# danielmtzbarba/carlabev-env

Hardware: AMD Instinct MI355X
Metric: env-steps/sec (whole node) at N_envs x 128x128 semantic obs (higher is better)
Workload: dtype f64 state / u8 frames; 1 GPU; ego-only empty scene (rt_no_traffic_v1), 4096 envs/GPU, 128x128 semantic 6-class; config_id=2, envs_per_gpu=4096, global_envs=4096, obs_size=128, obs_mode=bev_semantic, parallelism=env-sharded x1

## Files before the change

carlabev_env_amd/_lib.py:

```python
from __future__ import annotations

import ctypes
import os

HERE = os.path.dirname(os.path.abspath(__file__))
LIB_PATH = os.environ.get("CBEV_LIB") or os.path.join(HERE, "libcbev.so")

_P = ctypes.c_void_p
_I = ctypes.c_int
_I64 = ctypes.c_int64

_lib = None


class CbevError(RuntimeError):
    pass


def lib():
    global _lib
    if _lib is not None:
        return _lib
    if not os.path.exists(LIB_PATH):
        raise CbevError(f"{LIB_PATH} not built; run `python -m carlabev_env_amd.build` (hipcc, gfx950)")
# ... 31 lines not shown
    L.cbev_reset_terminated.restype = _I
    L.cbev_final_frames.argtypes = [_P, _P, _I, _I, _I, _P, _P, _P, _P, _P, _P]
    L.cbev_final_frames.restype = _I
    L.cbev_bank_cursor.argtypes = [_P, _P]
    L.cbev_bank_cursor.restype = _I
    L.cbev_reset_counts.argtypes = [_P, _P, _I]
    L.cbev_reset_counts.restype = _I
    L.cbev_bank_stride.argtypes = [_I]
    L.cbev_bank_stride.restype = _I
    L.cbev_set_deferred_reset.argtypes = [_P, _I]
    L.cbev_set_deferred_reset.restype = _I
    L.cbev_reset_pending.argtypes = [_P]
    L.cbev_reset_pending.restype = _I
    L.cbev_set_split_step.argtypes = [_P, _I]
    L.cbev_set_split_step.restype = _I
    L.cbev_flush.argtypes = [_P]
    L.cbev_flush.restype = _I
    L.cbev_expand_obs.argtypes = [_P, _P, _I, _I, _I, _I, _I, _P, _P, _P]
    L.cbev_expand_obs.restype = _I
    L.cbev_expand_obs_typed.argtypes = [_P, _P, _I, _I, _I, _I, _I, _P, _I, _P, _P]
    L.cbev_expand_obs_typed.restype = _I
    L.cbev_expand_obs_heads.argtypes = [_P, _P, _I, _I, _P, _I, _I, _P, _I, _P, _P]
    L.cbev_expand_obs_heads.restype = _I
    L.cbev_unpack_obs.argtypes = [_P, _P, _I, _I, _I, _P, _P]
    L.cbev_unpack_obs.restype = _I
    L.cbev_pack_frames.argtypes = [_P, _P, _I, _P, _P]
    L.cbev_pack_frames.restype = _I
    L.cbev_unpack_frames.argtypes = [_P, _P, _I, _P, _P]
    L.cbev_unpack_frames.restype = _I
    L.cbev_vector_obs.argtypes = [_P, _P, _I, _P, _P]
# ... 27 lines not shown
def check(rc: int, what: str = "cbev call"):
    if rc != 0:
        msg = lib().cbev_last_error().decode("utf-8", "replace")
        raise CbevError(f"{what} failed ({rc}): {msg}")


EXPORTED_SYMBOLS = ("cbev_abi_version", "cbev_params_size", "cbev_layout_of", "cbev_field_names", "cbev_last_error",
                    "cbev_create", "cbev_destroy", "cbev_set_map", "cbev_step", "cbev_reset", "cbev_bank_frames",
                    "cbev_reset_frames", "cbev_reset_masked", "cbev_reset_terminated", "cbev_bank_cursor",
                    "cbev_reset_counts", "cbev_bank_stride",
                    "cbev_set_deferred_reset", "cbev_reset_pending", "cbev_flush",
                    "cbev_expand_obs", "cbev_vector_obs", "cbev_set_fov_mask", "cbev_set_obs_size", "cbev_resize_obs", "cbev_profile", "cbev_profile_read",
                    "cbev_profile_raster", "cbev_error_flags", "cbev_set_episode_stats", "cbev_episode_slot",
                    "cbev_wall_clock_hz", "cbev_termination_count", "cbev_pack_frames", "cbev_unpack_frames",
                    "cbev_expand_obs_typed", "cbev_unpack_obs", "cbev_set_split_step", "cbev_step_repeat",
                    "cbev_step_masked", "cbev_step_heads", "cbev_expand_obs_heads", "cbev_final_frames")

REPEAT_MAX = 64

OBS_F32, OBS_F16, OBS_U8, OBS_BITS = 0, 1, 2, 3

ERR_ACTION_INDEX = 1
ERR_RASTER_WINDOW = 2
ERR_RETREAT_ROUTE = 4
```

carlabev_env_amd/csrc/cbev.hip:

```cpp
#include <hip/hip_runtime.h>
#include <math.h>
#include <stdarg.h>
#include <stdio.h>
#include <stdlib.h>
#include <string.h>

#include <algorithm>
#include <string>
#include <type_traits>
#include <vector>

#include "../../include/cbev.h"
#include "cbev_device.h"

__constant__ SgTables c_sg;

__device__ __forceinline__ void d_set_target_speed_mps(DRec& r, int a, double s) {
  s = d_pymax(0.0, s);
  RAD(r, CBEV_AD_T_SPEED_MPS, a) = s;
  RAD(r, CBEV_AD_T_SPEED, a) = s / CB_MPP;
}

__device__ __forceinline__ void d_bset(DRec& r, int a, int st, double speed_mps) {
  RAI(r, CBEV_AI_BSTATE, a) = st;
// ... 2830 lines not shown
        for (int b = 0; b < 4; ++b)
          if ((tm >> b) & 1u) *(uint32_t*)(g + o + 4 * b) = *(const uint32_t*)(l + o + 4 * b);
      }
    } else {
      const int w = j - nhd - nhi;
      *(uint32_t*)(g + K.L.vis + 4 * w) = *(const uint32_t*)(l + 16 * p.n0 + (K.L.vis - K.L.raw_x) + 4 * w);
    }
  }
}

template <bool WHOLE, EgoGate GATE = EgoGate::None, bool FIRST = false>
__device__ __forceinline__ void ego_tail(uint8_t* lds, uint8_t* __restrict__ recs, int n, int ne, int st_rb,
                                         int st_n0, int st_n, int st_raw_x, const KArgs& K,
                                         double* __restrict__ reward_out, uint8_t* __restrict__ term_out,
                                         uint8_t* __restrict__ trunc_out, int32_t* __restrict__ cause_out,
                                         float* __restrict__ info_out, EgoCarry& C, uint64_t frozen_in = 0ull) {
  constexpr bool GATED = GATE != EgoGate::None;
  constexpr bool ACCUM = GATE == EgoGate::Term || (GATE == EgoGate::Mask && !FIRST);
  const int e0 = staged_env0(blockIdx.x, ne, n);
  const int ne_eff = min(ne, n - e0);
  if (ne_eff <= 0) return;
  const EgoPack pk = ego_pack(K.L);
  const int nslot = WHOLE && K.C.actor_cap == 0 ? 2 : 1;
  const CollScratchLayout SL = coll_scratch_layout(K.C, K.L.vis_words);
  const EgoLds M = ego_lds(lds, nslot, ne, pk, SL);
  uint8_t* const scr = M.scr;
  HeroPre* const pre = M.pre;
  const int* const rrow = M.rrow;
  const int tid = threadIdx.x;
  const int lane = tid & 63, wave = __builtin_amdgcn_readfirstlane(tid >> 6);
  const cbev_params& P = K.P;
// ... 172 lines not shown
        }
        {
          double rx_ = ax - x, ry_ = ay - y;
          double rvx = avx - hvx, rvy = avy - hvy;
          double nrm = sqrt(rx_ * rx_ + ry_ * ry_);
          double rel = (rvx * rx_ + rvy * ry_) / (nrm + 1e-6);
          if (!(rel >= 0)) ts = fabs(nrm / rel);
        }
      }
      ((double*)(scr + k * SL.bytes + SL.ttcc))[a] = tc;
      ((double*)(scr + k * SL.bytes + SL.ttcs))[a] = ts;
    }
  }
  __syncthreads();
  CBEV_STAMP(1, 1);
  if (tid < ne_eff && !(GATED && ((frozen >> tid) & 1ull))) {
    const DRec r = rec(tid);
    CollPre cp = coll_reduce_serial(scr + tid * SL.bytes, SL, r.hi[CBEV_HI_NACT], r.hi[CBEV_HI_NRAW]);
    cp.spx = C.spx;
    cp.spy = C.spy;
    double rsum = 0.0;
    if (ACCUM) rsum = reward_out[e0 + tid];
    collide_env(K, r, e0 + tid, cp, reward_out, term_out, trunc_out, cause_out, info_out);
    if (ACCUM) reward_out[e0 + tid] = rsum + r.hd[CBEV_HD_REWARD];
    if (r.hi[CBEV_HI_TERM]) K.tcount[e0 + tid] = tc0 + 1u;
  } else if (GATE == EgoGate::Mask && FIRST && tid < ne_eff) {
    reward_out[e0 + tid] = 0.0;
  }
  __syncthreads();
  CBEV_STAMP(1, 2);
  if (!WHOLE) {
    ego_tail_out(lds, recs, e0, ne_eff, K, pk);
    CBEV_STAMP(1, 3);
    return;
  }
  if (GATED) {
    ego_stage_out_live(lds, recs, e0, ne_eff, K, pk, frozen);
    return;
  }
  ego_stage_out(slot, recs, e0, ne_eff, K, pk);
  if (C.rest_k >= 0) *(uint4*)(recs + (int64_t)(e0 + C.rest_k) * rb + C.rest_o) = C.rest_v;
  const int rsA = (int)((K.L.vis - K.L.cx) / 16), rsB0 = (int)(K.L.vis / 16) + pk.nvis;
  const int rpp = rsA + (int)(rb / 16) - rsB0, nres = __popcll(rbits);
  for (int q = threadIdx.x + 256; q < nres * rpp; q += 256) {
    const int k = nth_set_bit(rbits, q / rpp), c = q % rpp;
    const int o = c < rsA ? (int)K.L.cx + 16 * c : 16 * (rsB0 + c - rsA);
    *(uint4*)(recs + (int64_t)(e0 + k) * rb + o) = *(const uint4*)(src(k) + o);
// ... 69 lines not shown
  extern __shared__ __align__(16) uint8_t lds[];
  ego_mask_body<FIRST, false>(lds, recs, n, ne, st_rb, st_n0, st_n, st_raw_x, K, actions, active, reward_out, term_out,
                              trunc_out, cause_out, info_out, nullptr, 0);
}
__global__ __launch_bounds__(256) void k_ego_heads(uint8_t* __restrict__ recs, int n, int ne, int st_rb, int st_n0,
                                                   int st_n, int st_raw_x, KArgs K, const void* __restrict__ actions,
                                                   const uint8_t* __restrict__ active, double* __restrict__ reward_out,
                                                   uint8_t* __restrict__ term_out, uint8_t* __restrict__ trunc_out,
                                                   int32_t* __restrict__ cause_out, float* __restrict__ info_out,
                                                   uint8_t* __restrict__ heads, int n_frames) {
  extern __shared__ __align__(16) uint8_t lds[];
  ego_mask_body<true, true>(lds, recs, n, ne, st_rb, st_n0, st_n, st_raw_x, K, actions, active, reward_out, term_out,
                            trunc_out, cause_out, info_out, heads, n_frames);
}

__global__ __launch_bounds__(256) void k_ego_head(uint8_t* __restrict__ recs, int n, int ne, int st_rb, KArgs K,
                                                  const void* __restrict__ actions) {
  __shared__ double sh_pre[2][3][64];
  __shared__ float sh_act[3][64];
  CBEV_STAMP(0, 0);
  const int e0 = staged_env0(blockIdx.x, ne, n);
  const int ne_eff = min(ne, n - e0);
  if (ne_eff <= 0) return;
  const int tid = threadIdx.x;
  const int lane = tid & 63, wave = __builtin_amdgcn_readfirstlane(tid >> 6);
  const bool on = lane < ne_eff;
  const int e = e0 + (on ? lane : 0);
  const int vw = K.L.vis_words;
  const bool fold = K.rmask != nullptr;
  const uint8_t* const mp = fold ? K.rmask + e : recs;
  uint32_t mb = 0u, tc = 0u;
  double hd[CBEV_HD_COUNT] = {};
  int32_t hi[CBEV_HI_COUNT] = {};
  DRec r{};
  r.hd = hd;
  r.hi = hi;
  constexpr int NIN = 7;
  auto load_in = [&](const uint8_t* src, double* in) {
    const double* g = (const double*)(src + K.L.hd);
#pragma unroll
    for (int k = 0; k < 4; ++k) in[k] = g[CBEV_HD_X + k];
    in[4] = g[CBEV_HD_ACC];
    in[5] = g[CBEV_HD_TSPEED];
    in[6] = g[CBEV_HD_T];
  };
  auto chain = [&](int pass, const double* in) {
// ... 2 lines not shown
    hd[CBEV_HD_ACC] = in[4];
    hd[CBEV_HD_TSPEED] = in[5];
    hd[CBEV_HD_T] = in[6];
    HeroPre hp;
    hp.cyaw = sh_pre[pass][0][lane];
    hp.syaw = sh_pre[pass][1][lane];
    hp.tdelta = sh_pre[pass][2][lane];
    const float act3[3] = {sh_act[0][lane], sh_act[1][lane], sh_act[2][lane]};
    hero_env_phys(K, r, e, actions, hp, act3);
    hero_env_render_setup(K, r);
  };
  double in0[NIN] = {}, in1[NIN] = {}, v0 = 0.0, v1 = 0.0;
  float sa = 0.0f;
  const uint8_t* const own = recs + (int64_t)e * st_rb;
  if (wave == 0) {
    if (on) {
      load_in(own, in0);
      mb = *mp;
      tc = K.tcount[e];
      d_sincos(in0[2], &sh_pre[0][1][lane], &sh_pre[0][0][lane]);
    }
  } else if (wave == 1) {
    if (on) {
      v0 = ((const double*)(own + K.L.hd))[CBEV_HD_V];
      mb = *mp;
      tc = K.tcount[e];
      float g, b;
      d_decode_action(K, actions, e, &g, &sa, &b);
      sh_act[0][lane] = g;
      sh_act[1][lane] = sa;
      sh_act[2][lane] = b;
      sh_pre[0][2][lane] = hero_tan_delta(v0, sa);
    }
  } else {
    mb = *mp;
    tc = K.tcount[e];
    for (int q = tid - 128; q < ne_eff * vw; q += 128) {
      const int k = q / vw, w = q - k * vw;
      uint8_t* g = recs + (int64_t)(e0 + k) * st_rb + K.L.vis;
      const uint32_t v = ((const uint32_t*)g)[w];
      if (!(fold && K.rmask[e0 + k] != 0)) ((uint32_t*)g)[vw + w] = v;
    }
  }
  __syncthreads();
  CBEV_STAMP(0, 1);
  const bool reset = fold && on && mb != 0u;
  const uint64_t rbits = __ballot(reset);
  const int row = reset ? bank_row_of(e, tc, K.rstride, K.rn_bank) : 0;
  const uint8_t* const bank = K.rbank + (int64_t)row * st_rb;
  if (wave == 0 && reset) load_in(bank, in1);
  if (wave == 1 && reset) v1 = ((const double*)(bank + K.L.hd))[CBEV_HD_V];
  if (wave == 0 && on && !reset) chain(0, in0);
  if (rbits != 0ull) {
    if (wave == 0) {
      if (reset) {
#pragma unroll
        for (int k = 0; k < NIN; ++k) asm volatile("" : "+v"(in1[k]));
        d_sincos(in1[2], &sh_pre[1][1][lane], &sh_pre[1][0][lane]);
      }
    } else if (wave == 1) {
      if (reset) sh_pre[1][2][lane] = hero_tan_delta(v1, sa);
    } else {
      const int np = st_rb / 16, total = __popcll(rbits) * np;
      const int d0 = (int)K.L.vis + 4 * vw, d1 = d0 + 4 * vw;
      auto piece = [&](int q, const uint8_t** b, uint8_t** g, int* o) {
        const int j = q < total ? q / np : 0, k = nth_set_bit(rbits, j);
        *o = 16 * (q - j * np);
        *b = K.rbank + (int64_t)__shfl(row, k) * st_rb + *o;
        *g = recs + (int64_t)(e0 + k) * st_rb + *o;
      };
      auto by_word = [&](const uint8_t* b, uint8_t* g, int o) {
        for (int w = 0; w < 16; w += 4)
          *(uint32_t*)(g + w) = *(const uint32_t*)(b + w - (o + w >= d0 && o + w < d1 ? 4 * vw : 0));
      };
      for (int base = tid - 128; base - (tid - 128) < total; base += 256) {
        const uint8_t *b0, *b1;
        uint8_t *g0, *g1;
        int o0, o1;
        piece(base, &b0, &g0, &o0);
        piece(base + 128, &b1, &g1, &o1);
        const bool a0 = base < total, a1 = base + 128 < total;
        const bool w0 = o0 + 16 <= d0 || o0 >= d1, w1 = o1 + 16 <= d0 || o1 >= d1;
        uint4 x0 = make_uint4(0, 0, 0, 0), x1 = x0;
        if (a0 && w0) x0 = *(const uint4*)b0;
        if (a1 && w1) x1 = *(const uint4*)b1;
        if (a0 && w0) *(uint4*)g0 = x0;
        if (a1 && w1) *(uint4*)g1 = x1;
        if (a0 && !w0) by_word(b0, g0, o0);
        if (a1 && !w1) by_word(b1, g1, o1);
      }
    }
    __syncthreads();
    if (wave == 0 && reset) chain(1, in1);
  }
  CBEV_STAMP(0, 2);
  if (wave == 0 && on) {
    if (reset) {
      hi[CBEV_HI_RS_FAST] |= (row + 1) << 1;
      if (K.stats != nullptr) K.stats[e].t0 = (double)wall_clock64();
    }
    uint8_t* g = recs + (int64_t)e * st_rb;
    double* ohd = (double*)(g + K.L.hd);
    int32_t* ohi = (int32_t*)(g + K.L.hi);
#pragma unroll
    for (int k = 0; k < 8; k += 2) *(double2*)(ohd + CBEV_HD_X + k) = make_double2(hd[CBEV_HD_X + k], hd[CBEV_HD_X + k + 1]);
    ohd[CBEV_HD_ACC] = hd[CBEV_HD_ACC];
    *(double2*)(ohd + CBEV_HD_U_GAS) = make_double2(hd[CBEV_HD_U_GAS], hd[CBEV_HD_U_STEER]);
    *(double2*)(ohd + CBEV_HD_U_BRAKE) = make_double2(hd[CBEV_HD_U_BRAKE], hd[CBEV_HD_U_DELTA]);
    ohd[CBEV_HD_T] = hd[CBEV_HD_T];
#pragma unroll
    for (int k = CBEV_HI_RS_XMIN; k <= CBEV_HI_RS_FAST; ++k) ohi[k] = hi[k];
  }
  CBEV_STAMP(0, 3);
}
constexpr int HEAD_NE_DEFAULT = 16;
static_assert(CBEV_HD_X % 2 == 0 && CBEV_HD_U_GAS % 2 == 0 && CBEV_HD_U_BRAKE == CBEV_HD_U_GAS + 2 &&
                  CBEV_HD_U_DELTA == CBEV_HD_U_GAS + 3,
              "k_ego_head stores X .. V1 and U_* as 16-byte pieces");

struct TailArgs {
  int ntail;
  int ne, rb, n0, np, raw_x;
  double* reward;
  uint8_t* term;
  uint8_t* trunc;
  int32_t* cause;
  float* info;
};

struct RasterArgs {
  KArgs K;
  uint8_t* recs;
  int n;
  uint8_t* frames;
  TailArgs T;
};
template <int G>
__global__ __launch_bounds__(kRasterNT)
__attribute__((amdgpu_waves_per_eu(Tiles<G>::wgs_per_cu * kRasterNT / 256 > 8 ? 8 : Tiles<G>::wgs_per_cu * kRasterNT / 256)))
void k_raster(RasterArgs A) {
  extern __shared__ __align__(16) uint8_t lds[];
  if constexpr (G > 1) {
    if ((int)blockIdx.x < A.T.ntail) {
      const RasterArgs M = *(const RasterArgs*)__builtin_amdgcn_kernarg_segment_ptr();
      const TailArgs& T = M.T;
      EgoCarry C;
      ego_tail<false>(lds, M.recs, M.n, T.ne, T.rb, T.n0, T.np, T.raw_x, M.K, T.reward, T.term, T.trunc, T.cause,
                      T.info, C);
      return;
    }
  }
  const KArgs& K = A.K;
  uint8_t* __restrict__ const recs = A.recs;
  uint8_t* __restrict__ const frames = A.frames;
  const int n = A.n;
  const TailArgs& T = A.T;
  CBEV_STAMP(2, 0);
  int e, t;
  xcd_tile_of_wg((int)blockIdx.x - T.ntail, n, Tiles<G>::T, &e, &t);
  if (e >= n) return;
  const int64_t SS = (int64_t)K.P.size * K.P.size;
  const DRec r = bind_rec(recs + (int64_t)e * K.L.record_bytes, K.L, K.C);
  const RasterJob J = raster_job<false, G>(K, r);
// ... 416 lines not shown
  int defer_reset;
  struct {
    int on;
    void* records;
    int n;
    const uint8_t* mask;
    const void* bank;
    int n_bank;
    const uint8_t* bank_frames;
    uint8_t* frames;
    int n_frames;
    void* stream;
  } pend;
  const uint8_t* last_term;
  int last_n;
};

static int ego_ne_for(int per_env, int actor_cap) {
  const int budget = 128 * 1024;
  const char* v = getenv("CBEV_EGO_NE");
  int ne = v ? atoi(v) : (actor_cap <= 16 ? 16 : actor_cap <= 32 ? 8 : 4);
  ne = ne >= 64 ? 64 : ne >= 32 ? 32 : ne >= 16 ? 16 : ne >= 8 ? 8 : 4;
  while (ne > 4 && ne * per_env > budget) ne >>= 1;
  return ne * per_env > budget ? 0 : ne;
}

static int head_ne_for() {
  const char* v = getenv("CBEV_HEAD_NE");
  const int ne = v ? atoi(v) : HEAD_NE_DEFAULT;
  return ne >= 64 ? 64 : ne >= 32 ? 32 : ne >= 16 ? 16 : ne >= 8 ? 8 : 4;
// ... 174 lines not shown
  do {                                                                                                \
    if (!(c)->map_dev) return set_err(CBEV_ESTATE, "cbev_set_map not called");                        \
    if ((n) <= 0) return CBEV_OK;                                                                     \
    if ((c)->stats && (n) > (c)->ep_n)                                                                \
      return set_err(CBEV_EINVAL, "n %d exceeds the %d envs of the episode stats", (n), (c)->ep_n); \
  } while (0)

struct StepRun {
  KArgs K;
  hipStream_t s;
  hipEvent_t* ev;
};
static int step_begin(cbev_ctx* c, int n, uint8_t* term, void* stream, StepRun* R) {
  R->s = (hipStream_t)stream;
  R->K = kargs(c);
  c->last_term = term;
  c->last_n = n;
  if (n > c->seq_n) c->seq_n = n;
  if (c->stats) {
    const int slot = (int)(c->step_count % c->ep_ring), next = (slot + 1) % c->ep_ring;
    R->K.ep_rows = c->ep_rows + (int64_t)slot * c->ep_n * CBEV_EP_COUNT;
    R->K.ep_count = c->ep_counts + slot;
    R->K.ep_count_next = c->ep_counts + next;
    R->K.ep_cap = c->ep_n;
    c->step_count += 1;
  }
  R->ev = c->prof_on && c->prof_n < CBEV_PROF_MAX ? c->prof_ev + 4 * c->prof_n++ : nullptr;
  if (R->ev) HIP_TRY(hipEventRecord(R->ev[0], R->s));
  return CBEV_OK;
}
// ... 69 lines not shown
    return set_err(CBEV_EINVAL, "record layout: the k_ego staging ranges are not contiguous");
  if (ego_ne == 0)
    return set_err(CBEV_EINVAL, "k_ego stages 4 records per workgroup: %d bytes each do not fit its LDS budget",
                   per_env);
  HIP_TRY(hipSetDevice(device));
  cbev_ctx* c = (cbev_ctx*)calloc(1, sizeof(cbev_ctx));
  c->P = P;
  c->C = *caps;
  c->L = lay;
  c->device = device;
  c->ego_ne = ego_ne;
  c->ego_lb = ego_ne * per_env;
  c->tail_ne = tail_ne_for(P, *caps, lay, ego_ne);
  c->split = c->tail_ne > 0;
  c->head_ne = head_ne_for();
  SgTables T;
  build_sg_tables(&T);
  hipError_t e = hipMemcpyToSymbol(HIP_SYMBOL(c_sg), &T, sizeof T);
  if (e == hipSuccess) e = hipMalloc(&c->lut_dev, 64 * sizeof(uint32_t));
  if (e == hipSuccess) e = hipMalloc(&c->err_dev, sizeof(int32_t));
  if (e == hipSuccess) e = hipMemset(c->err_dev, 0, sizeof(int32_t));
  if (e == hipSuccess) e = hipMalloc(&c->nterm_dev, sizeof(unsigned long long));
  if (e == hipSuccess) e = hipMemset(c->nterm_dev, 0, sizeof(unsigned long long));
  const size_t seq_bytes = (size_t)CBEV_RESET_MASK_MAX_N * sizeof(uint32_t);
  if (e == hipSuccess) e = hipMalloc(&c->seq_dev, seq_bytes);
  if (e == hipSuccess) e = hipMemset(c->seq_dev, 0, seq_bytes);
  if (e == hipSuccess) {
    int khz = 0;
    e = hipDeviceGetAttribute(&khz, hipDeviceAttributeWallClockRate, device);
    c->tick_s = khz > 0 ? 1.0 / (1000.0 * khz) : 0.0;
  }
  if (e == hipSuccess) {
    const uint32_t pal[16] = CBEV_PALETTE_RGB;
    e = hipMemcpyToSymbol(HIP_SYMBOL(c_palette_rgb), pal, sizeof pal);
  }
  c->obs_h = c->obs_w = P.size;
  if (e == hipSuccess)
    e = hipFuncSetAttribute((const void*)k_ego, hipFuncAttributeMaxDynamicSharedMemorySize, c->ego_lb);
  if (e == hipSuccess)
    e = hipFuncSetAttribute((const void*)k_ego_rep, hipFuncAttributeMaxDynamicSharedMemorySize, c->ego_lb);
  if (e == hipSuccess)
// ... 135 lines not shown
void cbev_destroy(cbev_ctx* c) {
  if (!c) return;
  c->pend.on = 0;
  (void)hipSetDevice(c->device);
  if (c->prof_ev) {
    for (int i = 0; i < 4 * CBEV_PROF_MAX; ++i) (void)hipEventDestroy(c->prof_ev[i]);
    free(c->prof_ev);
  }
  if (c->map_dev) (void)hipFree(c->map_dev);
  if (c->map8_dev) (void)hipFree(c->map8_dev);
  if (c->map8T_dev) (void)hipFree(c->map8T_dev);
  if (c->lut_dev) (void)hipFree(c->lut_dev);
  if (c->err_dev) (void)hipFree(c->err_dev);
  if (c->nterm_dev) (void)hipFree(c->nterm_dev);
  if (c->seq_dev) (void)hipFree(c->seq_dev);
  if (c->area_dev) (void)hipFree(c->area_dev);
  if (c->fov_dev) (void)hipFree(c->fov_dev);
  free(c);
}

int cbev_set_map(cbev_ctx* c, const uint8_t* map_host, int64_t bytes) {
  if (!c || !map_host) return set_err(CBEV_EINVAL, "null argument");
  CBEV_FLUSH(c);
  const int64_t need = (int64_t)c->P.map_pitch * c->P.render_h;
  if (bytes != need) return set_err(CBEV_EINVAL, "map bytes %lld != pitch*render_h %lld", (long long)bytes, (long long)need);
  const int W = c->P.render_w, H = c->P.render_h, pitch = c->P.map_pitch;
  for (int64_t i = 0; i < need; ++i)
    if (map_host[i] > 15) return set_err(CBEV_EINVAL, "class id %d > 15 at byte %lld", map_host[i], (long long)i);
  const int np = ((W + 1) / 2 + 63) & ~63;
  std::vector<uint8_t> packed((size_t)np * H, 0);
// ... 28 lines not shown
  HIP_TRY(hipMemcpy(c->map8T_dev, map8T.data(), (size_t)p8T * W, hipMemcpyHostToDevice));
  c->p8T = p8T;
  return CBEV_OK;
}

int cbev_step(cbev_ctx* c, void* records, int n, const void* actions, uint8_t* frames, double* reward, uint8_t* term,
              uint8_t* trunc, int32_t* cause, float* info, void* stream) {
  if (!c || !records || !actions || !frames || !reward || !term || !trunc || !cause)
    return set_err(CBEV_EINVAL, "null argument");
  CBEV_STEP_CHECKS(c, n);
  const int64_t stride = (int64_t)n * c->P.size * c->P.size;
  const int64_t off = c->pend.on ? frames - c->pend.frames : 0;
  const bool fold = c->pend.on && records == c->pend.records && n == c->pend.n && off >= 0 && off % stride == 0 &&
                    off / stride < c->pend.n_frames && fold_ok(c, n);
  if (!fold) CBEV_FLUSH(c);
  StepRun R;
  const int rc = step_begin(c, n, term, stream, &R);
  if (rc != CBEV_OK) return rc;
  if (fold) {
    R.K.rmask = c->pend.mask;
    R.K.rbank = (const uint8_t*)c->pend.bank;
    R.K.rbank_frames = c->pend.bank_frames;
    R.K.rring = c->pend.frames;
    R.K.rring_stride = stride;
    R.K.rn_bank = c->pend.n_bank;
    R.K.rn_frames = c->pend.n_frames;
    R.K.rslot = (int)(off / stride);
    R.K.rstride = bank_stride(c->pend.n_bank);
    c->pend.on = 0;
  }
  launch_actors(c, actors_kernel(c->C), R, records, n);
  if (R.ev) HIP_TRY(hipEventRecord(R.ev[1], R.s));
  TailArgs T{};
  if (c->split) {
    hipLaunchKernelGGL(k_ego_head, dim3((n + c->head_ne - 1) / c->head_ne), dim3(256), 0, R.s, (uint8_t*)records, n,
                       c->head_ne, (int)c->L.record_bytes, R.K, actions);
    const EgoPack pk = ego_pack(c->L);
    T = TailArgs{((n + c->tail_ne - 1) / c->tail_ne + 7) & ~7, c->tail_ne, (int)c->L.record_bytes, pk.n0, pk.n,
                 (int)c->L.raw_x, reward, term, trunc, cause, info};
  } else {
    launch_ego(c, k_ego, R, records, n, actions, reward, term, trunc, cause, info);
  }
  if (R.ev) HIP_TRY(hipEventRecord(R.ev[2], R.s));
  launch_raster(c, CBEV_BY_SIZE(k_raster, c->P.size), n, T.ntail, R.s,
                RasterArgs{R.K, (uint8_t*)records, n, frames, T});
  return step_end(R);
}

enum StepKind { STEP_REPEAT, STEP_MASKED, STEP_HEADS };
struct StepChain {
  StepKind kind;
  const uint8_t *active, *prev_frames;
  uint8_t* heads;
  int n_frames;
// ... 99 lines not shown
  if (n <= 0) return CBEV_OK;
  KArgs K = kargs(c);
  const size_t lb = raster_lds_bytes(c->P);
  hipStream_t s = (hipStream_t)stream;
  const int grid = n < RESET_WGS ? n : RESET_WGS;
  hipLaunchKernelGGL(CBEV_BY_SIZE(k_reset, c->P.size), dim3(grid), dim3(256), lb, s, K, (uint8_t*)records, n,
                     (const uint8_t*)bank, n_bank, mask, bank_idx, bank_offset, frames, n_frames);
  HIP_TRY(hipGetLastError());
  return CBEV_OK;
}

int cbev_bank_frames(cbev_ctx* c, const void* bank, int n_bank, uint8_t* frames, void* stream) {
  if (!c || !bank || !frames) return set_err(CBEV_EINVAL, "null argument");
  CBEV_FLUSH(c);
  if (!c->map_dev) return set_err(CBEV_ESTATE, "cbev_set_map not called");
  if (n_bank <= 0) return CBEV_OK;
  KArgs K = kargs(c);
  const size_t lb = raster_lds_bytes(c->P);
  hipStream_t s = (hipStream_t)stream;
  const int grid = n_bank < RESET_WGS ? n_bank : RESET_WGS;
  hipLaunchKernelGGL(CBEV_BY_SIZE(k_bank_frames, c->P.size), dim3(grid), dim3(256), lb, s, K, (const uint8_t*)bank,
                     n_bank, frames);
  HIP_TRY(hipGetLastError());
  return CBEV_OK;
}

int cbev_reset_frames(cbev_ctx* c, void* records, int n, const void* bank, int n_bank, const uint8_t* mask,
                      const int32_t* bank_idx, int bank_offset, const uint8_t* bank_frames, uint8_t* frames,
                      int n_frames, void* stream) {
  if (!c || !records || !bank || !bank_frames || !frames) return set_err(CBEV_EINVAL, "null argument");
// ... 18 lines not shown
  if (n > CBEV_RESET_MASK_MAX_N) return set_err(CBEV_EINVAL, "n %d exceeds %d", n, CBEV_RESET_MASK_MAX_N);
  if (n <= 0) return CBEV_OK;
  CBEV_FLUSH(c);
  return launch_reset_mask(c, records, n, mask, bank, n_bank, bank_frames, frames, n_frames, stream);
}

static int launch_reset_mask(cbev_ctx* c, void* records, int n, const uint8_t* mask, const void* bank, int n_bank,
                             const uint8_t* bank_frames, uint8_t* frames, int n_frames, void* stream) {
  KArgs K = kargs(c);
  const int SS = c->P.size * c->P.size;
  const int64_t ppe = reset_pieces((int64_t)SS) + reset_pieces(c->L.record_bytes);
  const int64_t pieces = (int64_t)n * ppe;
  const int grid = pieces >= RESET_MASK_WGS ? RESET_MASK_WGS : (int)pieces;
  const int upt = reset_mask_upt(n);
  if (n > c->seq_n) c->seq_n = n;
  hipLaunchKernelGGL(k_reset_mask, dim3(grid), dim3(256), reset_mask_lds(n), (hipStream_t)stream, n, n_bank,
                     bank_stride(n_bank), (int)c->L.record_bytes, SS, n_frames, upt, mask, c->seq_dev,
                     (uint8_t*)records, (const uint8_t*)bank, bank_frames, frames, K);
  HIP_TRY(hipGetLastError());
  return CBEV_OK;
}

int cbev_reset_terminated(cbev_ctx* c, void* records, int n, const void* bank, int n_bank, const uint8_t* bank_frames,
                          uint8_t* frames, int n_frames, void* stream) {
  if (!c) return set_err(CBEV_EINVAL, "null argument");
  if (c->last_n == 0) return set_err(CBEV_ESTATE, "cbev_reset_terminated before any cbev_step");
  if (n != c->last_n) return set_err(CBEV_EINVAL, "n %d != the %d envs of the last cbev_step", n, c->last_n);
  if (c->defer_reset && fold_ok(c, n)) {
    if (!records || !bank || !bank_frames || !frames) return set_err(CBEV_EINVAL, "null argument");
    if (n_bank <= 0) return set_err(CBEV_EINVAL, "empty bank");
// ... 18 lines not shown
  if (!c) return set_err(CBEV_EINVAL, "null argument");
  if (!on) CBEV_FLUSH(c);
  c->defer_reset = on != 0;
  return CBEV_OK;
}

int cbev_reset_pending(const cbev_ctx* c) { return c && c->pend.on ? 1 : 0; }

int cbev_set_split_step(cbev_ctx* c, int on) {
  if (!c) return set_err(CBEV_EINVAL, "null argument");
  if (on && c->tail_ne == 0)
    return set_err(CBEV_EINVAL, "the split step is not supported at size %d with these capacities: k_ego's tail "
                                "does not fit k_raster's registers or its %zu bytes of LDS",
                   c->P.size, raster_lds_bytes(c->P));
  c->split = on != 0;
  return CBEV_OK;
}

int cbev_flush(cbev_ctx* c) {
  if (!c) return set_err(CBEV_EINVAL, "null argument");
  return flush_pending(c);
}

int cbev_bank_cursor(cbev_ctx* c, int64_t* cursor) {
  if (!c || !cursor) return set_err(CBEV_EINVAL, "null argument");
  CBEV_FLUSH(c);
  HIP_TRY(hipSetDevice(c->device));
  HIP_TRY(hipDeviceSynchronize());
  std::vector<uint32_t> v((size_t)c->seq_n);
  if (c->seq_n > 0) HIP_TRY(hipMemcpy(v.data(), c->seq_dev, v.size() * sizeof(uint32_t), hipMemcpyDeviceToHost));
// ... 382 lines not shown
```

carlabev_env_amd/csrc/cbev_device.h:

```cpp
#pragma once

#include <hip/hip_runtime.h>
#include <stdint.h>

#include "../../include/cbev_layout.h"

#define CB_DT 0.1
#define CB_WHEELBASE 2.9
#define CB_MPP 0.3125
#define CB_PI 3.141592653589793

struct KArgs {
  cbev_params P;
  cbev_caps C;
  cbev_layout L;
  const uint8_t* map;
  int npitch;
  const uint8_t* map8;
  int p8;
  const uint8_t* map8T;
  int p8T;
  const uint32_t* fov;
  int32_t* err;
  unsigned long long* nterm;
  cbev_episode_stats* stats;
  double* ep_rows;
  int32_t* ep_count;
  int32_t* ep_count_next;
  int ep_cap;
  double tick_s;
  uint32_t* tcount;
  const uint8_t* rmask;
  const uint8_t* rbank;
  const uint8_t* rbank_frames;
  uint8_t* rring;
  int64_t rring_stride;
  int rn_bank, rn_frames, rslot;
  uint32_t rstride;
};

__device__ __forceinline__ int d_map_texel(const KArgs& K, int x, int y) {
  return (K.map[(int64_t)y * K.npitch + (x >> 1)] >> ((x & 1) << 2)) & 15;
}

struct SgTables {
  double conv[6][11];
  double left[6][5][11];
  double right[6][5][11];
};
extern __constant__ SgTables c_sg;

struct DRec {
  double* hd;
// ... 225 lines not shown
```

include/cbev.h:

```cpp
#ifndef CBEV_H
#define CBEV_H

#include <stdint.h>

#include "cbev_layout.h"

#ifdef __cplusplus
extern "C" {
#endif

#define CBEV_ABI_VERSION 7

typedef struct cbev_ctx cbev_ctx;

enum { CBEV_OK = 0, CBEV_EINVAL = -1, CBEV_EHIP = -2, CBEV_ESTATE = -3 };

int cbev_abi_version(void);
int cbev_params_size(void);
int cbev_layout_of(const cbev_caps* caps, cbev_layout* out);
const char* cbev_field_names(int group);
const char* cbev_last_error(void);

int cbev_create(const cbev_params* params, const cbev_caps* caps, int device, cbev_ctx** out);
void cbev_destroy(cbev_ctx* ctx);
// ... 40 lines not shown
                      const uint8_t* bank_frames, uint8_t* frames, int n_frames, void* stream);
int cbev_reset_terminated(cbev_ctx* ctx, void* records, int n, const void* bank, int n_bank,
                          const uint8_t* bank_frames, uint8_t* frames, int n_frames, void* stream);
int cbev_final_frames(cbev_ctx* ctx, const uint8_t* ring, int n, int n_frames, int head, const uint8_t* heads,
                      const uint8_t* mask, uint8_t* out, int32_t* out_env, int32_t* out_count, void* stream);

int cbev_bank_cursor(cbev_ctx* ctx, int64_t* cursor);
int cbev_reset_counts(cbev_ctx* ctx, uint32_t* counts_host, int n);
int cbev_bank_stride(int n_bank);
int cbev_set_deferred_reset(cbev_ctx* ctx, int on);
int cbev_reset_pending(const cbev_ctx* ctx);
int cbev_flush(cbev_ctx* ctx);

int cbev_set_split_step(cbev_ctx* ctx, int on);

int cbev_expand_obs(cbev_ctx* ctx, const uint8_t* ring, int n, int n_frames, int head, int kind, int n_channels,
                    const uint32_t* channel_lut_host, void* out, void* stream);

#define CBEV_OBS_F32 0
#define CBEV_OBS_F16 1
#define CBEV_OBS_U8 2
#define CBEV_OBS_BITS 3
int cbev_expand_obs_typed(cbev_ctx* ctx, const uint8_t* ring, int n, int n_frames, int head, int kind, int n_channels,
                          const uint32_t* channel_lut_host, int out_dtype, void* out, void* stream);
int cbev_expand_obs_heads(cbev_ctx* ctx, const uint8_t* ring, int n, int n_frames, const uint8_t* heads, int kind,
                          int n_channels, const uint32_t* channel_lut_host, int out_dtype, void* out, void* stream);
int cbev_unpack_obs(cbev_ctx* ctx, const uint8_t* packed, int rows, int pixels, int out_dtype, void* out, void* stream);

int cbev_vector_obs(cbev_ctx* ctx, const void* records, int n, float* out, void* stream);

// ... 21 lines not shown
```

Baseline: 119.9 million env-steps/s.

## Preview reset-bank ego state in the tail so the next head skips reload

When an env terminates in the split-step tail, the tail now writes the bank row's ego head state (x, y, yaw, v, acc, target speed, t) into a 64-byte per-env preview slot tagged with the step serial, and a wave touches the bank row to warm the cache. On the next folded reset, k_ego_head<true> checks the tag and row, runs the kinematic chain directly from the previewed inputs, and skips the bank load and second sync for those envs. Head-state words are left out of the bank copy for all resets. This adds a preview buffer, atomic counters, template dispatch and tag bookkeeping, and depends on the preview staying consistent with the pending bank.

```diff
diff --git a/carlabev_env_amd/_lib.py b/carlabev_env_amd/_lib.py
--- a/carlabev_env_amd/_lib.py
+++ b/carlabev_env_amd/_lib.py
@@ -69,6 +69,10 @@
     L.cbev_reset_pending.restype = _I
     L.cbev_set_split_step.argtypes = [_P, _I]
     L.cbev_set_split_step.restype = _I
+    L.cbev_set_reset_preview.argtypes = [_P, _I]
+    L.cbev_set_reset_preview.restype = _I
+    L.cbev_reset_preview_counts.argtypes = [_P, _P]
+    L.cbev_reset_preview_counts.restype = _I
     L.cbev_flush.argtypes = [_P]
     L.cbev_flush.restype = _I
     L.cbev_expand_obs.argtypes = [_P, _P, _I, _I, _I, _I, _I, _P, _P, _P]
@@ -126,7 +130,8 @@
                     "cbev_profile_raster", "cbev_error_flags", "cbev_set_episode_stats", "cbev_episode_slot",
                     "cbev_wall_clock_hz", "cbev_termination_count", "cbev_pack_frames", "cbev_unpack_frames",
                     "cbev_expand_obs_typed", "cbev_unpack_obs", "cbev_set_split_step", "cbev_step_repeat",
-                    "cbev_step_masked", "cbev_step_heads", "cbev_expand_obs_heads", "cbev_final_frames")
+                    "cbev_step_masked", "cbev_step_heads", "cbev_expand_obs_heads", "cbev_final_frames",
+                    "cbev_set_reset_preview", "cbev_reset_preview_counts")
 
 REPEAT_MAX = 64
 
diff --git a/carlabev_env_amd/csrc/cbev.hip b/carlabev_env_amd/csrc/cbev.hip
--- a/carlabev_env_amd/csrc/cbev.hip
+++ b/carlabev_env_amd/csrc/cbev.hip
@@ -2868,7 +2868,8 @@
                                          int st_n0, int st_n, int st_raw_x, const KArgs& K,
                                          double* __restrict__ reward_out, uint8_t* __restrict__ term_out,
                                          uint8_t* __restrict__ trunc_out, int32_t* __restrict__ cause_out,
-                                         float* __restrict__ info_out, EgoCarry& C, uint64_t frozen_in = 0ull) {
+                                         float* __restrict__ info_out, EgoCarry& C, uint64_t frozen_in = 0ull,
+                                         const PvArgs* pvw = nullptr) {
   constexpr bool GATED = GATE != EgoGate::None;
   constexpr bool ACCUM = GATE == EgoGate::Term || (GATE == EgoGate::Mask && !FIRST);
   const int e0 = staged_env0(blockIdx.x, ne, n);
@@ -3071,6 +3072,8 @@
   }
   __syncthreads();
   CBEV_STAMP(1, 1);
+  int trow1 = 0;
+  uint32_t touched = 0u;
   if (tid < ne_eff && !(GATED && ((frozen >> tid) & 1ull))) {
     const DRec r = rec(tid);
     CollPre cp = coll_reduce_serial(scr + tid * SL.bytes, SL, r.hi[CBEV_HI_NACT], r.hi[CBEV_HI_NRAW]);
@@ -3080,14 +3083,47 @@
     if (ACCUM) rsum = reward_out[e0 + tid];
     collide_env(K, r, e0 + tid, cp, reward_out, term_out, trunc_out, cause_out, info_out);
     if (ACCUM) reward_out[e0 + tid] = rsum + r.hd[CBEV_HD_REWARD];
-    if (r.hi[CBEV_HI_TERM]) K.tcount[e0 + tid] = tc0 + 1u;
+    if (r.hi[CBEV_HI_TERM]) {
+      K.tcount[e0 + tid] = tc0 + 1u;
+      if (GATE == EgoGate::None && pvw != nullptr && K.rbank != nullptr && pvw->tag != 0u) {
+        const int row = bank_row_of(e0 + tid, tc0 + 1u, K.rstride, K.rn_bank);
+        const double* g = (const double*)(K.rbank + (int64_t)row * st_rb + K.L.hd);
+        RPreview* const pv = pvw->pv + (e0 + tid);
+        const double x = g[CBEV_HD_X], y = g[CBEV_HD_Y], yaw = g[CBEV_HD_YAW], v = g[CBEV_HD_V];
+        const double acc = g[CBEV_HD_ACC], ts = g[CBEV_HD_TSPEED], t = g[CBEV_HD_T];
+        double2* const o = (double2*)pv;
+        o[0] = make_double2(x, y);
+        o[1] = make_double2(yaw, v);
+        o[2] = make_double2(acc, ts);
+        union {
+          uint32_t u[2];
+          double d;
+        } w;
+        w.u[0] = (uint32_t)row + 1u;
+        w.u[1] = pvw->tag;
+        o[3] = make_double2(t, w.d);
+        trow1 = row + 1;
+      }
+    }
   } else if (GATE == EgoGate::Mask && FIRST && tid < ne_eff) {
     reward_out[e0 + tid] = 0.0;
+  }
+  if (!WHOLE && GATE == EgoGate::None && wave == 0 && pvw != nullptr && K.rbank != nullptr && pvw->tag != 0u) {
+    uint32_t t0 = 0u, t1 = 0u;
+    for (uint64_t tb = __ballot(trow1 != 0); tb != 0ull; tb &= tb - 1ull) {
+      const int row = __shfl(trow1, __builtin_ctzll(tb)) - 1;
+      const uint8_t* const b = K.rbank + (int64_t)row * st_rb;
+      t0 |= *(const uint32_t*)(b + min(128 * lane, st_rb - 4));
+      t1 |= *(const uint32_t*)(b + st_rb - 4);
+      for (int o = 128 * (64 + lane); o < st_rb; o += 128 * 64) t1 |= *(const uint32_t*)(b + o);
+    }
+    touched = t0 | t1;
   }
   __syncthreads();
   CBEV_STAMP(1, 2);
   if (!WHOLE) {
     ego_tail_out(lds, recs, e0, ne_eff, K, pk);
+    asm volatile("" ::"v"(touched));
     CBEV_STAMP(1, 3);
     return;
   }
@@ -3187,9 +3223,11 @@
                             trunc_out, cause_out, info_out, heads, n_frames);
 }
 
+template <bool PV>
 __global__ __launch_bounds__(256) void k_ego_head(uint8_t* __restrict__ recs, int n, int ne, int st_rb, KArgs K,
-                                                  const void* __restrict__ actions) {
+                                                  const void* __restrict__ actions, PvArgs V) {
   __shared__ double sh_pre[2][3][64];
+  __shared__ double sh_pin[7][64];
   __shared__ float sh_act[3][64];
   CBEV_STAMP(0, 0);
   const int e0 = staged_env0(blockIdx.x, ne, n);
@@ -3199,10 +3237,21 @@
   const int lane = tid & 63, wave = __builtin_amdgcn_readfirstlane(tid >> 6);
   const bool on = lane < ne_eff;
   const int e = e0 + (on ? lane : 0);
-  const int vw = K.L.vis_words;
-  const bool fold = K.rmask != nullptr;
-  const uint8_t* const mp = fold ? K.rmask + e : recs;
+  const uint8_t* rmask = K.rmask;
+  const RPreview* pvb = V.pv;
+  const uint32_t* tcnt = K.tcount;
+  int vw = K.L.vis_words;
+  asm volatile("" : "+s"(rmask), "+s"(pvb), "+s"(tcnt), "+s"(vw));
+  const bool fold = rmask != nullptr;
+  const uint8_t* const mp = fold ? rmask + e : recs;
+  const RPreview* const pt = pvb + (fold ? e : 0);
   uint32_t mb = 0u, tc = 0u;
+  uint2 ptag = make_uint2(0u, 0u);
+  const int pvl = PV && 2 * ne <= 64 ? ne : 0;
+  const int kp = lane - pvl;
+  const bool isp = PV && kp >= 0 && kp < ne_eff;
+  const RPreview* const pp = pvb + (fold ? e0 + (isp ? kp : 0) : 0);
+  const int nround = !PV || pvl ? 1 : 2;
   double hd[CBEV_HD_COUNT] = {};
   int32_t hi[CBEV_HI_COUNT] = {};
   DRec r{};
@@ -3235,32 +3284,75 @@
   float sa = 0.0f;
   const uint8_t* const own = recs + (int64_t)e * st_rb;
   if (wave == 0) {
-    if (on) {
+    if (PV || on) {
+      const double2* const q = (const double2*)pp;
+      const double2 o23 = *(const double2*)((const double*)(own + K.L.hd) + CBEV_HD_YAW);
+      double2 p01 = make_double2(0.0, 0.0), p23 = p01, p45 = p01;
+      double p6 = 0.0;
+      if (PV) p23 = q[1];
       load_in(own, in0);
+      in0[2] = o23.x;
+      in0[3] = o23.y;
       mb = *mp;
-      tc = K.tcount[e];
-      d_sincos(in0[2], &sh_pre[0][1][lane], &sh_pre[0][0][lane]);
+      tc = tcnt[e];
+      if (PV) {
+        ptag = *(const uint2*)&pt->row1;
+        p01 = q[0];
+        p45 = q[2];
+        p6 = pp->in[6];
+      }
+#pragma unroll 1
+      for (int it = 0; it < nround; ++it) {
+        const bool pr = pvl ? lane >= pvl : it == 1;
+        const int k = pr ? kp : lane;
+        double sn, cs;
+        d_sincos(pr ? p23.x : in0[2], &sn, &cs);
+        if (k >= 0 && k < ne_eff) {
+          sh_pre[pr][1][k] = sn;
+          sh_pre[pr][0][k] = cs;
+        }
+      }
+      if (isp) {
+        sh_pin[0][kp] = p01.x;
+        sh_pin[1][kp] = p01.y;
+        sh_pin[2][kp] = p23.x;
+        sh_pin[3][kp] = p23.y;
+        sh_pin[4][kp] = p45.x;
+        sh_pin[5][kp] = p45.y;
+        sh_pin[6][kp] = p6;
+      }
     }
   } else if (wave == 1) {
-    if (on) {
+    if (PV || on) {
       v0 = ((const double*)(own + K.L.hd))[CBEV_HD_V];
       mb = *mp;
-      tc = K.tcount[e];
+      tc = tcnt[e];
+      if (PV) ptag = *(const uint2*)&pt->row1;
+      const double pv3 = PV ? pp->in[3] : 0.0;
       float g, b;
-      d_decode_action(K, actions, e, &g, &sa, &b);
-      sh_act[0][lane] = g;
-      sh_act[1][lane] = sa;
-      sh_act[2][lane] = b;
-      sh_pre[0][2][lane] = hero_tan_delta(v0, sa);
+      d_decode_action(K, actions, pvl && isp ? e0 + kp : e, &g, &sa, &b);
+      if (on) {
+        sh_act[0][lane] = g;
+        sh_act[1][lane] = sa;
+        sh_act[2][lane] = b;
+      }
+#pragma unroll 1
+      for (int it = 0; it < nround; ++it) {
+        const bool pr = pvl ? lane >= pvl : it == 1;
+        const int k = pr ? kp : lane;
+        const double td = hero_tan_delta(pr ? pv3 : v0, sa);
+        if (k >= 0 && k < ne_eff) sh_pre[pr][2][k] = td;
+      }
     }
   } else {
     mb = *mp;
-    tc = K.tcount[e];
+    tc = tcnt[e];
+    if (PV) ptag = *(const uint2*)&pt->row1;
     for (int q = tid - 128; q < ne_eff * vw; q += 128) {
       const int k = q / vw, w = q - k * vw;
       uint8_t* g = recs + (int64_t)(e0 + k) * st_rb + K.L.vis;
       const uint32_t v = ((const uint32_t*)g)[w];
-      if (!(fold && K.rmask[e0 + k] != 0)) ((uint32_t*)g)[vw + w] = v;
+      if (!(fold && rmask[e0 + k] != 0)) ((uint32_t*)g)[vw + w] = v;
     }
   }
   __syncthreads();
@@ -3268,22 +3360,41 @@
   const bool reset = fold && on && mb != 0u;
   const uint64_t rbits = __ballot(reset);
   const int row = reset ? bank_row_of(e, tc, K.rstride, K.rn_bank) : 0;
+  const bool fast = PV && reset && V.acc != 0u && ptag.y == V.acc && ptag.x == (uint32_t)row + 1u;
+  const bool slow = reset && !fast;
+  const uint64_t sbits = __ballot(slow);
   const uint8_t* const bank = K.rbank + (int64_t)row * st_rb;
-  if (wave == 0 && reset) load_in(bank, in1);
-  if (wave == 1 && reset) v1 = ((const double*)(bank + K.L.hd))[CBEV_HD_V];
-  if (wave == 0 && on && !reset) chain(0, in0);
+  if (wave == 0 && slow) load_in(bank, in1);
+  if (wave == 1 && slow) v1 = ((const double*)(bank + K.L.hd))[CBEV_HD_V];
+  if (wave == 0 && on && !slow) {
+    if (fast) {
+#pragma unroll
+      for (int k = 0; k < NIN; ++k) in0[k] = sh_pin[k][lane];
+    }
+    chain(fast ? 1 : 0, in0);
+  }
   if (rbits != 0ull) {
     if (wave == 0) {
-      if (reset) {
+      if (slow) {
 #pragma unroll
         for (int k = 0; k < NIN; ++k) asm volatile("" : "+v"(in1[k]));
         d_sincos(in1[2], &sh_pre[1][1][lane], &sh_pre[1][0][lane]);
       }
     } else if (wave == 1) {
-      if (reset) sh_pre[1][2][lane] = hero_tan_delta(v1, sa);
+      if (slow) sh_pre[1][2][lane] = hero_tan_delta(v1, sa);
     } else {
       const int np = st_rb / 16, total = __popcll(rbits) * np;
       const int d0 = (int)K.L.vis + 4 * vw, d1 = d0 + 4 * vw;
+      const int hd0 = (int)K.L.hd, hi0 = (int)K.L.hi;
+      auto head_word = [&](int o) {
+        const int d = (o - hd0) >> 3, i = (o - hi0) >> 2;
+        const bool h = o >= hd0 && ((d >= CBEV_HD_X && d < CBEV_HD_X + 8) || d == CBEV_HD_ACC ||
+                                    (d >= CBEV_HD_U_GAS && d < CBEV_HD_U_GAS + 4) || d == CBEV_HD_T);
+        return h || (o >= hi0 && i >= CBEV_HI_RS_XMIN && i <= CBEV_HI_RS_FAST);
+      };
+      auto whole = [&](int o) {
+        return (o + 16 <= d0 || o >= d1) && !(head_word(o) || head_word(o + 4) || head_word(o + 8) || head_word(o + 12));
+      };
       auto piece = [&](int q, const uint8_t** b, uint8_t** g, int* o) {
         const int j = q < total ? q / np : 0, k = nth_set_bit(rbits, j);
         *o = 16 * (q - j * np);
@@ -3291,8 +3402,12 @@
         *g = recs + (int64_t)(e0 + k) * st_rb + *o;
       };
       auto by_word = [&](const uint8_t* b, uint8_t* g, int o) {
-        for (int w = 0; w < 16; w += 4)
-          *(uint32_t*)(g + w) = *(const uint32_t*)(b + w - (o + w >= d0 && o + w < d1 ? 4 * vw : 0));
+        uint32_t x[4];
+#pragma unroll
+        for (int w = 0; w < 4; ++w) x[w] = *(const uint32_t*)(b + 4 * w - (o + 4 * w >= d0 && o + 4 * w < d1 ? 4 * vw : 0));
+#pragma unroll
+        for (int w = 0; w < 4; ++w)
+          if (!head_word(o + 4 * w)) *(uint32_t*)(g + 4 * w) = x[w];
       };
       for (int base = tid - 128; base - (tid - 128) < total; base += 256) {
         const uint8_t *b0, *b1;
@@ -3301,7 +3416,7 @@
         piece(base, &b0, &g0, &o0);
         piece(base + 128, &b1, &g1, &o1);
         const bool a0 = base < total, a1 = base + 128 < total;
-        const bool w0 = o0 + 16 <= d0 || o0 >= d1, w1 = o1 + 16 <= d0 || o1 >= d1;
+        const bool w0 = whole(o0), w1 = whole(o1);
         uint4 x0 = make_uint4(0, 0, 0, 0), x1 = x0;
         if (a0 && w0) x0 = *(const uint4*)b0;
         if (a1 && w1) x1 = *(const uint4*)b1;
@@ -3311,15 +3426,19 @@
         if (a1 && !w1) by_word(b1, g1, o1);
       }
     }
-    __syncthreads();
-    if (wave == 0 && reset) chain(1, in1);
+    if (sbits != 0ull) {
+      __syncthreads();
+      if (wave == 0 && slow) chain(1, in1);
+    }
   }
   CBEV_STAMP(0, 2);
   if (wave == 0 && on) {
     if (reset) {
       hi[CBEV_HI_RS_FAST] |= (row + 1) << 1;
       if (K.stats != nullptr) K.stats[e].t0 = (double)wall_clock64();
-    }
+      if (V.cnt != nullptr) atomicAdd(V.cnt + (fast ? 0 : 1), 1ull);
+    }
+    if (PV && fold && V.acc != 0u && ptag.y == V.acc) V.pv[e].tag = 0u;
     uint8_t* g = recs + (int64_t)e * st_rb;
     double* ohd = (double*)(g + K.L.hd);
     int32_t* ohi = (int32_t*)(g + K.L.hi);
@@ -3347,6 +3466,7 @@
   uint8_t* trunc;
   int32_t* cause;
   float* info;
+  PvArgs pv;
 };
 
 struct RasterArgs {
@@ -3367,7 +3487,7 @@
       const TailArgs& T = M.T;
       EgoCarry C;
       ego_tail<false>(lds, M.recs, M.n, T.ne, T.rb, T.n0, T.np, T.raw_x, M.K, T.reward, T.term, T.trunc, T.cause,
-                      T.info, C);
+                      T.info, C, 0ull, &T.pv);
       return;
     }
   }
@@ -3814,6 +3934,13 @@
   } pend;
   const uint8_t* last_term;
   int last_n;
+  RPreview* pv_dev;
+  unsigned long long* pvcnt_dev;
+  int pv_on;
+  uint32_t serial;
+  int pv_live;
+  const void* pv_bank;
+  int pv_n_bank;
 };
 
 static int ego_ne_for(int per_env, int actor_cap) {
@@ -4018,6 +4145,8 @@
 static int step_begin(cbev_ctx* c, int n, uint8_t* term, void* stream, StepRun* R) {
   R->s = (hipStream_t)stream;
   R->K = kargs(c);
+  if (++c->serial == 0u) c->serial = 1u;
+  c->pv_live = 0;
   c->last_term = term;
   c->last_n = n;
   if (n > c->seq_n) c->seq_n = n;
@@ -4117,6 +4246,7 @@
   c->tail_ne = tail_ne_for(P, *caps, lay, ego_ne);
   c->split = c->tail_ne > 0;
   c->head_ne = head_ne_for();
+  c->pv_on = c->split && caps->actor_cap == 0;
   SgTables T;
   build_sg_tables(&T);
   hipError_t e = hipMemcpyToSymbol(HIP_SYMBOL(c_sg), &T, sizeof T);
@@ -4128,6 +4258,12 @@
   const size_t seq_bytes = (size_t)CBEV_RESET_MASK_MAX_N * sizeof(uint32_t);
   if (e == hipSuccess) e = hipMalloc(&c->seq_dev, seq_bytes);
   if (e == hipSuccess) e = hipMemset(c->seq_dev, 0, seq_bytes);
+  const size_t pv_bytes = (size_t)CBEV_RESET_MASK_MAX_N * sizeof(RPreview);
+  const bool pv_can = c->tail_ne > 0 && caps->actor_cap == 0;
+  if (pv_can && e == hipSuccess) e = hipMalloc(&c->pv_dev, pv_bytes);
+  if (pv_can && e == hipSuccess) e = hipMemset(c->pv_dev, 0, pv_bytes);
+  if (pv_can && e == hipSuccess) e = hipMalloc(&c->pvcnt_dev, 2 * sizeof(unsigned long long));
+  if (pv_can && e == hipSuccess) e = hipMemset(c->pvcnt_dev, 0, 2 * sizeof(unsigned long long));
   if (e == hipSuccess) {
     int khz = 0;
     e = hipDeviceGetAttribute(&khz, hipDeviceAttributeWallClockRate, device);
@@ -4293,6 +4429,8 @@
   if (c->err_dev) (void)hipFree(c->err_dev);
   if (c->nterm_dev) (void)hipFree(c->nterm_dev);
   if (c->seq_dev) (void)hipFree(c->seq_dev);
+  if (c->pv_dev) (void)hipFree(c->pv_dev);
+  if (c->pvcnt_dev) (void)hipFree(c->pvcnt_dev);
   if (c->area_dev) (void)hipFree(c->area_dev);
   if (c->fov_dev) (void)hipFree(c->fov_dev);
   free(c);
@@ -4351,10 +4489,21 @@
   const bool fold = c->pend.on && records == c->pend.records && n == c->pend.n && off >= 0 && off % stride == 0 &&
                     off / stride < c->pend.n_frames && fold_ok(c, n);
   if (!fold) CBEV_FLUSH(c);
+  const uint32_t pvacc = fold && c->pv_on && c->split && c->pv_live && c->pv_bank == c->pend.bank && c->pv_n_bank == c->pend.n_bank
+                             ? c->serial
+                             : 0u;
+  PvArgs V{c->pv_dev, c->pvcnt_dev, 0u, 0u};
   StepRun R;
   const int rc = step_begin(c, n, term, stream, &R);
   if (rc != CBEV_OK) return rc;
   if (fold) {
+    if (c->pv_on && c->split) {
+      V.acc = pvacc;
+      V.tag = c->serial;
+      c->pv_live = 1;
+      c->pv_bank = c->pend.bank;
+      c->pv_n_bank = c->pend.n_bank;
+    }
     R.K.rmask = c->pend.mask;
     R.K.rbank = (const uint8_t*)c->pend.bank;
     R.K.rbank_frames = c->pend.bank_frames;
@@ -4370,11 +4519,11 @@
   if (R.ev) HIP_TRY(hipEventRecord(R.ev[1], R.s));
   TailArgs T{};
   if (c->split) {
-    hipLaunchKernelGGL(k_ego_head, dim3((n + c->head_ne - 1) / c->head_ne), dim3(256), 0, R.s, (uint8_t*)records, n,
-                       c->head_ne, (int)c->L.record_bytes, R.K, actions);
+    hipLaunchKernelGGL(V.acc != 0u ? k_ego_head<true> : k_ego_head<false>, dim3((n + c->head_ne - 1) / c->head_ne),
+                       dim3(256), 0, R.s, (uint8_t*)records, n, c->head_ne, (int)c->L.record_bytes, R.K, actions, V);
     const EgoPack pk = ego_pack(c->L);
     T = TailArgs{((n + c->tail_ne - 1) / c->tail_ne + 7) & ~7, c->tail_ne, (int)c->L.record_bytes, pk.n0, pk.n,
-                 (int)c->L.raw_x, reward, term, trunc, cause, info};
+                 (int)c->L.raw_x, reward, term, trunc, cause, info, V};
   } else {
     launch_ego(c, k_ego, R, records, n, actions, reward, term, trunc, cause, info);
   }
@@ -4504,6 +4653,8 @@
   if (!c || !bank || !frames) return set_err(CBEV_EINVAL, "null argument");
   CBEV_FLUSH(c);
   if (!c->map_dev) return set_err(CBEV_ESTATE, "cbev_set_map not called");
+  c->pv_live = 0;
+  if (c->pv_dev && c->seq_n > 0) HIP_TRY(hipMemsetAsync(c->pv_dev, 0, (size_t)c->seq_n * sizeof(RPreview), (hipStream_t)stream));
   if (n_bank <= 0) return CBEV_OK;
   KArgs K = kargs(c);
   const size_t lb = raster_lds_bytes(c->P);
@@ -4552,6 +4703,7 @@
   const int grid = pieces >= RESET_MASK_WGS ? RESET_MASK_WGS : (int)pieces;
   const int upt = reset_mask_upt(n);
   if (n > c->seq_n) c->seq_n = n;
+  c->pv_live = 0;
   hipLaunchKernelGGL(k_reset_mask, dim3(grid), dim3(256), reset_mask_lds(n), (hipStream_t)stream, n, n_bank,
                      bank_stride(n_bank), (int)c->L.record_bytes, SS, n_frames, upt, mask, c->seq_dev,
                      (uint8_t*)records, (const uint8_t*)bank, bank_frames, frames, K);
@@ -4600,6 +4752,28 @@
                                 "does not fit k_raster's registers or its %zu bytes of LDS",
                    c->P.size, raster_lds_bytes(c->P));
   c->split = on != 0;
+  return CBEV_OK;
+}
+
+int cbev_set_reset_preview(cbev_ctx* c, int on) {
+  if (!c) return set_err(CBEV_EINVAL, "null argument");
+  if (on && (c->tail_ne == 0 || c->C.actor_cap != 0))
+    return set_err(CBEV_EINVAL, "the reset preview needs the split step and the folded reset: size %d, %d actor slots",
+                   c->P.size, c->C.actor_cap);
+  c->pv_on = on != 0;
+  c->pv_live = 0;
+  return CBEV_OK;
+}
+
+int cbev_reset_preview_counts(cbev_ctx* c, uint64_t out[2]) {
+  if (!c || !out) return set_err(CBEV_EINVAL, "null argument");
+  CBEV_FLUSH(c);
+  HIP_TRY(hipSetDevice(c->device));
+  HIP_TRY(hipDeviceSynchronize());
+  unsigned long long v[2] = {0, 0};
+  if (c->pvcnt_dev) HIP_TRY(hipMemcpy(v, c->pvcnt_dev, sizeof v, hipMemcpyDeviceToHost));
+  out[0] = v[0];
+  out[1] = v[1];
   return CBEV_OK;
 }
 
diff --git a/carlabev_env_amd/csrc/cbev_device.h b/carlabev_env_amd/csrc/cbev_device.h
--- a/carlabev_env_amd/csrc/cbev_device.h
+++ b/carlabev_env_amd/csrc/cbev_device.h
@@ -37,6 +37,18 @@
   int64_t rring_stride;
   int rn_bank, rn_frames, rslot;
   uint32_t rstride;
+};
+
+struct __attribute__((aligned(64))) RPreview {
+  double in[7];
+  uint32_t row1;
+  uint32_t tag;
+};
+static_assert(sizeof(RPreview) == 64, "a preview entry is one 64-byte piece");
+struct PvArgs {
+  RPreview* pv;
+  unsigned long long* cnt;
+  uint32_t tag, acc;
 };
 
 __device__ __forceinline__ int d_map_texel(const KArgs& K, int x, int y) {
diff --git a/include/cbev.h b/include/cbev.h
--- a/include/cbev.h
+++ b/include/cbev.h
@@ -78,6 +78,9 @@
 
 int cbev_set_split_step(cbev_ctx* ctx, int on);
 
+int cbev_set_reset_preview(cbev_ctx* ctx, int on);
+int cbev_reset_preview_counts(cbev_ctx* ctx, uint64_t out[2]);
+
 int cbev_expand_obs(cbev_ctx* ctx, const uint8_t* ring, int n, int n_frames, int head, int kind, int n_channels,
                     const uint32_t* channel_lut_host, void* out, void* stream);
 
```

New measurement: 122.3 million env-steps/s, median of 6. 2.0% higher.
